# lionl1106/Searchable-Generative-Image-Compression

Measured on AMD Instinct MI355X. Metric: images/sec end-to-end compress (enc+entropy+CLIP) at 256x256, higher is better.
Workload: dtype f32; 1 GPU; configs[1]: batch=32 256x256 encoder+entropy+CLIP compress per GPU, TiTok ViT-L hybrid encoder + ViT-B/32 CLIP, synthetic weights; global_batch=32

## Files before the change

### include/sgic.h

```cpp
#ifndef SGIC_H
#define SGIC_H
#include <stddef.h>
#include <stdint.h>

#ifdef __cplusplus
extern "C" {
#endif

typedef struct ihipStream_t *sgic_stream_t;

#define SGIC_OK 0
#define SGIC_EINVAL -1
#define SGIC_EHIP -2
#define SGIC_ENOSPC -3
#define SGIC_ENODEV -4

const char *sgic_last_error(void);
int sgic_version(void);
int sgic_device_count(void);


int sgic_pmf_to_quantized_cdf(const float *pmf, int n, int precision, uint32_t *cdf_out);

typedef struct sgic_cdf_table sgic_cdf_table;
// ... 38 lines not shown
  int attn_mode;
  sgic_profiler *profiler;
  int w_packed;
  int a_packed;
} sgic_launch_opts;

int sgic_profiler_create(sgic_profiler **out);
void sgic_profiler_destroy(sgic_profiler *p);
int sgic_profiler_begin(sgic_profiler *p, int max_launches);
int sgic_profiler_end(sgic_profiler *p, float *ms_out, int cap, int *n_out);

int sgic_gemm_f32(const float *d_A, int lda, const float *d_W, int ldw, const float *d_bias, const float *d_R,
                  int ldr, float *d_C, int ldc, int M, int N, int K, int act, int a_seg, int a_seg_stride,
                  int c_seg, int c_seg_stride, const sgic_launch_opts *opts, sgic_stream_t stream);

int sgic_layernorm_f32(const float *d_x, int ldx, int xseg, int xseg_stride, const float *d_gamma,
                       const float *d_beta, float *d_y, int ldy, int yseg, int yseg_stride, int M, int C, float eps,
                       int act, sgic_stream_t stream);

int sgic_attention_f32(const float *d_q, int ldq, const float *d_k, int ldk, const float *d_v, int ldv,
                       float *d_out, int ldo, int L, int nseq, int nheads, const int32_t *d_rowmap,
                       const float *d_bias, const int32_t *d_biasvar, float scale, const sgic_launch_opts *opts,
                       sgic_stream_t stream);

int sgic_im2col_patch(const float *d_x, int B, int C, int H, int W, int P, float mul, float add, int tile16,
                      float *d_out, sgic_stream_t stream);
int sgic_assemble_tokens(const float *d_emb, const float *d_cls, const float *d_pos, const float *d_lat,
                         const float *d_latpos, int N, int P, int T, int D, float *d_out, sgic_stream_t stream);
int sgic_add_rows_bcast(const float *d_in, int ldi, int iseg, const float *d_vec, float *d_out, int ldo, int oseg,
                        int Nn, int Lr, int D, sgic_stream_t stream);
int sgic_dwconv_nhwc(const float *d_x, const float *d_w, const float *d_bias, const float *d_prescale, float *d_y,
                     int B, int H, int W, int C, int k, int tile16, sgic_stream_t stream);
int sgic_im2col_2x2(const float *d_x, int B, int H, int W, int C, int tile16, float *d_out, sgic_stream_t stream);
int sgic_gated_lrelu(const float *d_x, float *d_out, int M, int C2, sgic_stream_t stream);
int sgic_colop(const float *d_x, int ldx, const float *d_v, int ldv, int vrows, float *d_y, int ldy, int M, int C,
               int mode, sgic_stream_t stream);
int sgic_fake2d_transpose(const float *d_in, long in_seq_stride, float *d_out, int N, int T, int D,
                          sgic_stream_t stream);
int sgic_vq_argmin(const float *d_z, int ldz, const float *d_codebook, int ncodes, int dim, int M, int l2norm,
                   int32_t *d_idx, sgic_stream_t stream);
int sgic_clip_preprocess(const float *d_x, long img_stride, long ch_stride, int ldx, int B, int H, int W, int OH,
                         int OW, int S, int top, int left, const int32_t *d_bounds_h, const int32_t *d_kk_h,
                         int ksize_h, const int32_t *d_bounds_v, const int32_t *d_kk_v, int ksize_v,
                         const float *mean3, const float *std3, uint8_t *d_tmp_u8, uint8_t *d_tmp_h, float *d_out,
                         sgic_stream_t stream);
int sgic_l2norm_u8(const float *d_x, int ldx, int M, int D, float *d_unit, uint8_t *d_q, sgic_stream_t stream);

int sgic_split3_f32(const float *d_x, int ld, int rows, int cols, int seg, int seg_stride, uint16_t *d_planes,
                    sgic_stream_t stream);
int sgic_split3_pack_f32(const float *d_x, int ld, int rows, int cols, uint16_t *d_planes, sgic_stream_t stream);
int sgic_gemm_split3_f32(const float *d_A, int lda, int a_seg, int a_seg_stride, uint16_t *d_Aplanes,
                         const uint16_t *d_Wplanes, const float *d_bias, const float *d_R, int ldr, float *d_C, int ldc,
                         uint16_t *d_Cplanes, int M, int N, int K, int act, int c_seg, int c_seg_stride,
                         const sgic_launch_opts *opts, sgic_stream_t stream);
int sgic_conv3x3_split3_f32(const uint16_t *d_in_planes, const uint16_t *d_Wplanes, const float *d_bias, const float *d_R,
                            int ldr, float *d_out, int ldc, int B, int H, int W, int Cin, int Cout, int act,
                            const sgic_launch_opts *opts, sgic_stream_t stream);
int sgic_groupnorm_nhwc_split3(const float *d_x, const float *d_gamma, const float *d_beta, int B, int H, int W, int C,
                               int groups, float eps, int swish, double *d_ws, float *d_stats, uint16_t *d_halo_planes,
                               sgic_stream_t stream);
int sgic_halo_copy_split3(const float *d_in, int B, int H, int W, int C, int upsample2x, int tile16, uint16_t *d_halo_planes,
                          sgic_stream_t stream);
int sgic_attention_split3_f32(const float *d_q, int ldq, const float *d_k, int ldk, const float *d_v, int ldv,
                              uint16_t *d_out_planes, long rows, int L, int nseq, int nheads, const int32_t *d_rowmap,
                              const float *d_bias, const int32_t *d_biasvar, float scale, const sgic_launch_opts *opts,
                              sgic_stream_t stream);
int sgic_layernorm_split3_f32(const float *d_x, int ldx, int xseg, int xseg_stride, const float *d_gamma,
                              const float *d_beta, uint16_t *d_planes, int M, int C, float eps, int act,
                              sgic_stream_t stream);

int sgic_gemm_batched_f32(const float *d_A, int lda, long strideA, const float *d_W, int ldw, long strideW,
                          const float *d_bias, const float *d_R, int ldr, long strideR, float *d_C, int ldc,
                          long strideC, int M, int N, int K, int act, int batch, const sgic_launch_opts *opts,
                          sgic_stream_t stream);
int sgic_conv3x3_f32(const float *d_in_halo, const float *d_W, const float *d_bias, const float *d_R, int ldr,
                     float *d_out, int ldc, int B, int H, int W, int Cin, int Cout, int act, const sgic_launch_opts *opts,
                     sgic_stream_t stream);
int sgic_groupnorm_nhwc(const float *d_x, const float *d_gamma, const float *d_beta, int B, int H, int W, int C,
                        int groups, float eps, int swish, int halo_out, double *d_ws, float *d_stats, float *d_y,
                        sgic_stream_t stream);
int sgic_halo_copy(const float *d_in, int B, int H, int W, int C, int upsample2x, int tile16, float *d_out,
                   sgic_stream_t stream);
int sgic_softmax_rows(const float *d_x, float *d_y, long M, int L, float scale, sgic_stream_t stream);
int sgic_pixel_shuffle2_tm16(const float *d_in, int B, int H, int W, int C, float *d_out, sgic_stream_t stream);
int sgic_assemble_dec_tokens(const float *d_emb, const float *d_cls, const float *d_mask, const float *d_pos,
                             const float *d_latpos, int N, int P, int T, int D, float *d_out, sgic_stream_t stream);
int sgic_codebook_gather_norm(const int32_t *d_idx, const float *d_codebook, int M, int dim, int ld, float *d_out,
                              sgic_stream_t stream);
int sgic_nhwc3_to_nchw_clamp(const float *d_in, int ld, int B, int H, int W, float *d_out, sgic_stream_t stream);
// ... 50 lines not shown
```

### searchable-generative-image-compression_amd/clip.py

```python
import math

import numpy as np
import torch

from . import ops
from ._lib import call
from .config import ClipConfig
from .encoder import RabW, rab_forward

_PREC = 22


def _bicubic(x):
    a = -0.5
    x = abs(x)
    if x < 1.0:
        return ((a + 2.0) * x - (a + 3.0)) * x * x + 1
    if x < 2.0:
        return (((x - 5) * x + 8) * x - 4) * a
    return 0.0


def pil_coeffs(in_size, out_size):
    scale = in_size / out_size
    fscale = max(scale, 1.0)
    support = 2.0 * fscale
    ksize = int(math.ceil(support)) * 2 + 1
    bounds = np.zeros((out_size, 2), dtype=np.int32)
    kk = np.zeros((out_size, ksize), dtype=np.int32)
    ss = 1.0 / fscale
    for xx in range(out_size):
# ... 5 lines not shown
        w = [_bicubic((x + xmin - center + 0.5) * ss) for x in range(xmax)]
        ww = 0.0
        for v in w:
            ww += v
        if ww != 0.0:
            w = [v / ww for v in w]
        for x, v in enumerate(w):
            kk[xx, x] = int(-0.5 + v * (1 << _PREC)) if v < 0 else int(0.5 + v * (1 << _PREC))
        bounds[xx] = (xmin, xmax)
    return bounds, kk, ksize


def resize_geometry(H, W, S):
    if H <= W:
        OH, OW = S, int(S * W / H)
    else:
        OH, OW = int(S * H / W), S
    top = int(round((OH - S) / 2.0))
    left = int(round((OW - S) / 2.0))
    return OH, OW, top, left


class ClipHIP:
    def __init__(self, sd, cfg: ClipConfig, device, p="clip.visual"):
        self.cfg, self.device = cfg, device
        g = lambda k: sd[f"{p}.{k}"].to(device=device, dtype=torch.float32).contiguous()
        Wd = cfg.width
        self.conv_w = sd[f"{p}.conv1.weight"].reshape(Wd, -1).to(device).contiguous()
        self.cls = g("class_embedding").reshape(1, Wd).contiguous()
        self.pos = g("positional_embedding")
        self.lnpre_w, self.lnpre_b = g("ln_pre.weight"), g("ln_pre.bias")
        self.blocks = [RabW(sd, f"{p}.transformer.resblocks.{i}", device) for i in range(cfg.layers)]
        self.lnpost_w, self.lnpost_b = g("ln_post.weight"), g("ln_post.bias")
        self.projT = sd[f"{p}.proj"].t().to(device).contiguous()
        self.mean = np.asarray(cfg.mean, dtype=np.float32)
        self.std = np.asarray(cfg.std, dtype=np.float32)
        self._coef = {}

    def _coeffs(self, H, W):
        key = (H, W)
        if key not in self._coef:
            S = self.cfg.image_size
            OH, OW, top, left = resize_geometry(H, W, S)
            bh, kh, ksh = pil_coeffs(W, OW)
            bv, kv, ksv = pil_coeffs(H, OH)
            d = lambda a: torch.from_numpy(np.ascontiguousarray(a)).to(self.device)
            self._coef[key] = (OH, OW, top, left, d(bh), d(kh), ksh, d(bv), d(kv), ksv)
        return self._coef[key]
# ... 31 lines not shown
             self.mean, self.std, ops._p(work), ctypes.c_size_t(nbytes.value), ops._p(out))
        return out

    def preprocess_u8(self, canvas, hw):
        if canvas.dim() != 4 or canvas.shape[3] != 3 or canvas.dtype != torch.uint8:
            raise ValueError(f"canvas must be (B, Hc, Wc, 3) uint8, got {tuple(canvas.shape)} {canvas.dtype}")
        B, Hc, Wc, _ = canvas.shape
        hw = np.asarray(hw, dtype=np.int64).reshape(B, 2)
        if (hw <= 0).any() or (hw[:, 0] > Hc).any() or (hw[:, 1] > Wc).any():
            raise ValueError(f"extents {hw.tolist()} outside the {Hc}x{Wc} canvas")
        S = self.cfg.image_size
        geo = np.array([(h, w) + resize_geometry(h, w, S) for h, w in hw.tolist()], dtype=np.int32)
        return ops.clip_preprocess_u8canvas(canvas.contiguous(), geo, S, self.mean, self.std)

    def tower(self, pre):
        cfg = self.cfg
        B = pre.shape[0]
        g = cfg.image_size // cfg.patch
        L = g * g + 1
        A = ops.im2col_patch(pre, cfg.patch, 1.0, 0.0, tile16=False)
        emb = ops.gemm(A, self.conv_w)
        X = ops.assemble_tokens(emb, self.cls, self.pos, None, None, B, g * g, 0, cfg.width)
        ops.layernorm(X, self.lnpre_w, self.lnpre_b, out=X)
        for w in self.blocks:
            rab_forward(X, w, L, B, cfg.heads)
        pooled = ops.layernorm(X, self.lnpost_w, self.lnpost_b, M=B, x_seg=(1, L))
        z = ops.gemm(pooled, self.projT)
        return ops.l2norm_u8(z)

    def encode(self, x, H=None, W=None, hw=None):
        return self.tower(self.preprocess(x, H, W, hw))

    def encode_u8(self, canvas, hw):
        return self.tower(self.preprocess_u8(canvas, hw))


class ClipTextHIP:

    def __init__(self, sd, cfg: ClipConfig, device, p="clip"):
        self.cfg, self.device = cfg, device
        g = lambda k: sd[f"{p}.{k}"].to(device=device, dtype=torch.float32).contiguous()
        self.table, self.pos = g("token_embedding.weight"), g("positional_embedding")
        self.blocks = [RabW(sd, f"{p}.transformer.resblocks.{i}", device) for i in range(cfg.t_layers)]
        self.lnf_w, self.lnf_b = g("ln_final.weight"), g("ln_final.bias")
        self.projT = sd[f"{p}.text_projection"].t().to(device=device, dtype=torch.float32).contiguous()
        L = self.L = (cfg.ctx + 3) & ~3
        if L != cfg.ctx:
            self.pos = torch.cat([self.pos, torch.zeros(L - cfg.ctx, cfg.t_width, device=device)]).contiguous()
        self.causal = torch.full((L, L), float("-inf")).triu_(1).reshape(1, L, L).to(device).contiguous()
# ... 20 lines not shown
```

### searchable-generative-image-compression_amd/csrc/attn.hip

```cpp
#include "common.h"
#include "split3.h"

typedef float f32x16 __attribute__((ext_vector_type(16)));
typedef float f32x4 __attribute__((ext_vector_type(4)));

#define AT_KT 32
#define AT_LOG2E 1.4426950408889634f
#define AT_DEFER 6.0f
#define AT_LDK 68
#define AT_LDV 64
#define AT_TILE (AT_KT * AT_LDK + AT_KT * AT_LDV)
#define AT_K3_ROWB 144
#define AT_K3_FLOATS (3 * AT_KT * AT_K3_ROWB / 4)
#define AT_V3_ROWB 80
#define AT_V3_FLOATS (3 * 64 * AT_V3_ROWB / 4)
typedef __bf16 at_bf16x8 __attribute__((ext_vector_type(8)));
typedef unsigned at_u32x4 __attribute__((ext_vector_type(4)));
typedef unsigned at_u32x2 __attribute__((ext_vector_type(2)));
#define AT_RAG_MAXL 960
#define AT_RAG_SLICE (64 + AT_RAG_MAXL)

#ifdef AT_STAMPS
__device__ long long at_stamps[4 * (1 << 17)];
__device__ long long at_real[2 * (1 << 17)];
// ... 9 lines not shown
#define AT_STAMP(i)
#endif

struct AttnArgs {
  const float *q, *k, *v;
  float *out;
  int ldq, ldk, ldv, ldo;
  int L, nseq, nheads;
  const int *rowmap;
  const float *bias;
  const int *biasvar;
  float scale;
  int nq;
  int ipw;
  int nqp;
  int n_items;
  int n_wgs;
  int group;
  int rag;
  int n_rag_wgs;
  int stagger_cycles, first_round;
  unsigned short *out_planes;
  long plane_elems;
};

__device__ __forceinline__ long at_row(const AttnArgs &a, int seq, int tok) {
  return a.rowmap ? (long)a.rowmap[(long)seq * a.L + tok] : (long)seq * a.L + tok;
}

__device__ void attn_ragged_row(const AttnArgs &a, int unit, int tok, float *wl , int lane) {
  const int head = unit % a.nheads, seq = unit / a.nheads, hc = head * 64;
  const long q_row = at_row(a, seq, tok);
  float *ql = wl, *pl = wl + 64;
  ql[lane] = a.q[q_row * a.ldq + hc + lane] * a.scale;
  const float *bias_row = nullptr;
  if (a.bias) bias_row = a.bias + ((long)(a.biasvar ? a.biasvar[seq] : 0) * a.L + tok) * a.L;
  float mx = -INFINITY;
  for (int key = lane; key < a.L; key += 64) {
    const float *kp = a.k + at_row(a, seq, key) * a.ldk + hc;
    float sc = 0.f;
#pragma unroll
    for (int c = 0; c < 16; c += 4) {
      f32x4 k4[4];
#pragma unroll
      for (int j = 0; j < 4; j++) k4[j] = *reinterpret_cast<const f32x4 *>(kp + (c + j) * 4);
#pragma unroll
      for (int j = 0; j < 4; j++) {
        const f32x4 q4 = *reinterpret_cast<const f32x4 *>(ql + (c + j) * 4);
#pragma unroll
        for (int t = 0; t < 4; t++) sc = fmaf(k4[j][t], q4[t], sc);
      }
    }
    if (bias_row) sc += bias_row[key];
    pl[key] = sc;
    mx = fmaxf(mx, sc);
// ... 27 lines not shown
    s3_split_pair(res, 0.f, p1, p2, p3);
    const size_t dst = s3_pack_off(q_row, hc + lane, a.plane_elems / (a.nheads * 64));
    a.out_planes[dst] = (unsigned short)p1;
    a.out_planes[a.plane_elems + dst] = (unsigned short)p2;
    a.out_planes[2 * a.plane_elems + dst] = (unsigned short)p3;
  } else {
    a.out[q_row * a.ldo + hc + lane] = res;
  }
}

static_assert(4 * AT_RAG_SLICE <= AT_TILE, "ragged-row slices must fit the smallest LDS configuration");

template <int NBUF, int UP, bool S3>
__global__ __launch_bounds__(256, (NBUF * UP >= 4 || (S3 && UP > 1)) ? 2 : 3) void attn_f32_kernel(AttnArgs a) {
  constexpr int KF = S3 ? AT_K3_FLOATS : AT_KT * AT_LDK;
  constexpr int VF = S3 ? AT_V3_FLOATS : AT_KT * AT_LDV;
  constexpr int TILE = KF + VF;
  __shared__ __attribute__((aligned(16))) float smem[NBUF * UP * TILE];
  const int tid = threadIdx.x, lane = tid & 63, wave = tid >> 6;

  int p = blockIdx.x;
  if (p < a.n_rag_wgs) {
    const int it = p * 4 + wave, n_units = a.nseq * a.nheads;
    if (it < n_units * a.rag) attn_ragged_row(a, it / a.rag, a.nq * 32 + it % a.rag, smem + wave * AT_RAG_SLICE, lane);
    return;
  }
  p -= a.n_rag_wgs;
  const int wg = (((p >> 3) / a.group) * 8 + (p & 7)) * a.group + (p >> 3) % a.group;
  if (wg >= a.n_wgs) return;

  if (a.stagger_cycles > 0 && p < a.first_round) {
    const unsigned slot = __builtin_amdgcn_s_getreg((3 << 11) | 4) & 7u;
    const unsigned s0 = __builtin_amdgcn_readfirstlane(slot);
    if (s0 > 0) {
      const long long t_end = (long long)__builtin_amdgcn_s_memtime() + (long long)s0 * a.stagger_cycles;
      while ((long long)__builtin_amdgcn_s_memtime() < t_end) __builtin_amdgcn_s_sleep(32);
    }
  }

  AT_STAMP(0);
  const int item0 = wg * a.ipw;
  const int uA = item0 / a.nqp;
  const int last = min(item0 + a.ipw, a.n_items) - 1;
  const bool two = UP > 1 && (last / a.nqp) != uA;
  const int item = item0 + wave;
  const int unit_i = item / a.nqp, rb_i = item - unit_i * a.nqp;
  const bool active = wave < a.ipw && item < a.n_items && rb_i < a.nq;
  const int unit = active ? unit_i : uA;
  const int rb = active ? rb_i : 0;
  const int mine = (UP > 1 && unit != uA) ? 1 : 0;
  const int head = unit % a.nheads, seq = unit / a.nheads;

  const int lq = lane & 31, lh = lane >> 5;
  const int q_tok = rb * 32 + lq;
  const bool q_ok = active && q_tok < a.L;
  const int q_tok_c = q_tok < a.L ? q_tok : a.L - 1;
  const long q_row = at_row(a, seq, q_tok_c);
  const int hc = head * 64;

  float qf[S3 ? 1 : 32];
  at_bf16x8 q3[S3 ? 4 : 1][3];
  {
    const float *qp = a.q + q_row * a.ldq + hc;
    if constexpr (S3) {
#pragma unroll
      for (int c = 0; c < 4; c++) {
        const f32x4 v0 = *reinterpret_cast<const f32x4 *>(qp + 16 * c + 8 * lh), v1 = *reinterpret_cast<const f32x4 *>(qp + 16 * c + 8 * lh + 4);
        at_u32x4 p1, p2, p3;
        unsigned a0, b0, c0;
        const float qs = a.scale * AT_LOG2E;
        s3_split_pair(v0[0] * qs, v0[1] * qs, a0, b0, c0); p1[0] = a0, p2[0] = b0, p3[0] = c0;
        s3_split_pair(v0[2] * qs, v0[3] * qs, a0, b0, c0); p1[1] = a0, p2[1] = b0, p3[1] = c0;
        s3_split_pair(v1[0] * qs, v1[1] * qs, a0, b0, c0); p1[2] = a0, p2[2] = b0, p3[2] = c0;
        s3_split_pair(v1[2] * qs, v1[3] * qs, a0, b0, c0); p1[3] = a0, p2[3] = b0, p3[3] = c0;
        q3[c][0] = __builtin_bit_cast(at_bf16x8, p1);
        q3[c][1] = __builtin_bit_cast(at_bf16x8, p2);
        q3[c][2] = __builtin_bit_cast(at_bf16x8, p3);
      }
    } else {
#pragma unroll
// ... 334 lines not shown
#pragma unroll
      for (int t = 0; t < 4; t++) w0[t] = o0[g4 * 4 + t] * inv, w1[t] = o1[g4 * 4 + t] * inv;
      if (a.out_planes) {
        const size_t prows = a.plane_elems / (a.nheads * 64);
        const size_t dst = s3_pack_off(q_row, hc + d, prows);
        s3_store4(a.out_planes, a.plane_elems, dst, w0);
        s3_store4(a.out_planes, a.plane_elems, dst + prows * 32, w1);
      } else {
        *reinterpret_cast<f32x4 *>(op + d) = w0;
        *reinterpret_cast<f32x4 *>(op + 32 + d) = w1;
      }
    }
  }
  AT_STAMP(3);
}

template <typename K>
static inline void launch_attn(K kernel, unsigned grid, hipStream_t st, const AttnArgs &a) {
  kernel<<<grid, 256, 0, st>>>(a);
}

static int attention_any(const float *d_q, int ldq, const float *d_k, int ldk, const float *d_v, int ldv, float *d_out, int ldo,
                         uint16_t *d_planes, long plane_rows, int L, int nseq, int nheads, const int32_t *d_rowmap,
                         const float *d_bias, const int32_t *d_biasvar, float scale, const sgic_launch_opts *opts,
                         sgic_stream_t stream) {
  SGIC_REQUIRE(d_q && d_k && d_v && (d_out || d_planes) && L > 0 && nseq > 0 && nheads > 0, "args");
  SGIC_REQUIRE((ldq & 3) == 0 && (ldk & 3) == 0 && (ldv & 3) == 0 && (ldo & 3) == 0, "row strides must be multiples of 4");
  SGIC_REQUIRE(ldq >= nheads * 64 && ldk >= nheads * 64 && ldv >= nheads * 64 && (d_planes || ldo >= nheads * 64), "head_dim is 64");
  SGIC_REQUIRE((((uintptr_t)d_q | (uintptr_t)d_k | (uintptr_t)d_v | (uintptr_t)d_out) & 15) == 0 && ((uintptr_t)d_planes & 7) == 0, "16-byte alignment");
  SGIC_REQUIRE(!d_planes || plane_rows >= (long)nseq * L, "plane rows");
  SGIC_REQUIRE(!d_bias || (L & 3) == 0, "bias needs L % 4 == 0");
  const int mode_all = opts ? opts->attn_mode : 0;
  SGIC_REQUIRE(mode_all >= 0 && mode_all <= 15, "attn_mode 0..7 (+8)");
  const bool s3 = (mode_all & 8) != 0;
  const int mode = mode_all & 7;
  const long units = (long)nseq * nheads;
  const int rem = L % 32;
  const int rag = (rem >= 1 && rem <= 2 && L >= 64 && L <= AT_RAG_MAXL) ? rem : 0;
  const int nq = rag ? L / 32 : (L + 31) / 32;
  const bool three = mode == 7 && nq >= 2;
  const int ipw = three ? 3 : (nq == 1 ? 2 : 4);
  const int nqp = three ? (nq + 2) / 3 * 3 : nq;
  const long n_items = units * nqp;
  SGIC_REQUIRE(n_items < (1l << 30), "too many (sequence, head, row block) items");
  const int n_wgs = (int)((n_items + ipw - 1) / ipw);
  const int group = (4 * nqp) / ipw;
  const long groups = (n_wgs + group - 1) / group;
  const long grid_mfma = ((groups + 7) / 8) * 8 * group;
  const int n_rag_wgs = (int)((units * rag + 3) / 4);
  const bool up2 = (nqp % ipw) != 0;
  AttnArgs a{d_q, d_k, d_v, d_out, ldq, ldk, ldv, ldo, L, nseq, nheads, d_rowmap, d_bias, d_biasvar, scale,
             nq, ipw, nqp, (int)n_items, n_wgs, group, rag, n_rag_wgs, 0, 0, d_planes, plane_rows * nheads * 64};
  const unsigned grid = (unsigned)(grid_mfma + n_rag_wgs);
  hipStream_t st = to_stream(stream);
  const int eff = three ? 1 : (mode ? (mode == 7 ? 1 : mode) : (up2 ? 5 : 1));
  const bool single = (eff & 1) != 0;
  a.stagger_cycles = eff > 2 ? 4096 * ((eff - 1) / 2) : 0;
  const int per_cu = (!single && up2) ? 2 : 3;
  a.first_round = per_cu * 256;
  if (s3) {
    if (up2) {
      if (single) launch_attn(attn_f32_kernel<1, 2, true>, grid, st, a);
      else launch_attn(attn_f32_kernel<2, 2, true>, grid, st, a);
    } else {
      if (single) launch_attn(attn_f32_kernel<1, 1, true>, grid, st, a);
      else launch_attn(attn_f32_kernel<2, 1, true>, grid, st, a);
    }
  } else if (up2) {
    if (single) launch_attn(attn_f32_kernel<1, 2, false>, grid, st, a);
    else launch_attn(attn_f32_kernel<2, 2, false>, grid, st, a);
  } else {
    if (single) launch_attn(attn_f32_kernel<1, 1, false>, grid, st, a);
    else launch_attn(attn_f32_kernel<2, 1, false>, grid, st, a);
  }
  return sgic::check_launch("attn_f32_kernel");
}

extern "C" int sgic_attention_f32(const float *d_q, int ldq, const float *d_k, int ldk, const float *d_v, int ldv,
                                  float *d_out, int ldo, int L, int nseq, int nheads, const int32_t *d_rowmap,
                                  const float *d_bias, const int32_t *d_biasvar, float scale, const sgic_launch_opts *opts,
                                  sgic_stream_t stream) {
  SGIC_REQUIRE(d_out, "out");
  return attention_any(d_q, ldq, d_k, ldk, d_v, ldv, d_out, ldo, nullptr, 0, L, nseq, nheads, d_rowmap, d_bias, d_biasvar, scale,
                       opts, stream);
}

extern "C" int sgic_attention_split3_f32(const float *d_q, int ldq, const float *d_k, int ldk, const float *d_v, int ldv,
                                         uint16_t *d_out_planes, long rows, int L, int nseq, int nheads,
                                         const int32_t *d_rowmap, const float *d_bias, const int32_t *d_biasvar, float scale,
                                         const sgic_launch_opts *opts, sgic_stream_t stream) {
  SGIC_REQUIRE(d_out_planes, "planes");
  return attention_any(d_q, ldq, d_k, ldk, d_v, ldv, nullptr, 0, d_out_planes, rows, L, nseq, nheads, d_rowmap, d_bias, d_biasvar,
                       scale, opts, stream);
}
```

### searchable-generative-image-compression_amd/csrc/misc.hip

```cpp
#include "common.h"
#include <limits.h>

typedef float f32x4 __attribute__((ext_vector_type(4)));

__device__ __forceinline__ long fmap_row(int b, int y, int x, int H, int W, int tile16) {
  if (!tile16) return ((long)b * H + y) * W + x;
  const int nH = H >> 4, nW = W >> 4;
  return ((((long)b * nH + (y >> 4)) * nW + (x >> 4)) << 8) + ((y & 15) << 4) + (x & 15);
}

#define GRID_STRIDE(i, n) for (long i = (long)blockIdx.x * blockDim.x + threadIdx.x; i < (n); i += (long)gridDim.x * blockDim.x)
static inline unsigned ew_grid(long n) {
  long g = (n + 255) / 256;
  return (unsigned)(g < 1 ? 1 : (g > 8192 ? 8192 : g));
}

__global__ void im2col_patch_kernel(const float *__restrict__ x, int B, int C, int H, int W, int P, float mul, float add,
                                    int tile16, float *__restrict__ out) {
  const int gh = H / P, gw = W / P, K = C * P * P, P4 = P >> 2;
  const long total = (long)B * gh * gw * C * P * P4;
  GRID_STRIDE(i, total) {
    long t = i;
    const int kx4 = (int)(t % P4);
    t /= P4;
// ... 242 lines not shown
  SGIC_REQUIRE(d_x && d_v && d_y && M > 0 && C > 0 && (C & 3) == 0 && vrows > 0 && (mode >= 0 && mode <= 2), "args");
  SGIC_REQUIRE((ldx & 3) == 0 && (ldv & 3) == 0 && (ldy & 3) == 0, "leading dims multiple of 4");
  colop_kernel<<<ew_grid((long)M * C / 4), 256, 0, to_stream(stream)>>>(d_x, ldx, d_v, ldv, vrows, d_y, ldy, M, C, mode);
  return sgic::check_launch("colop_kernel");
}

__global__ void fake2d_transpose_kernel(const float *__restrict__ in, long in_seq_stride, float *__restrict__ out, int N,
                                        int T, int D) {
  const long total = (long)N * T * D;
  GRID_STRIDE(i, total) {
    const int c = (int)(i % D);
    const long r = i / D;
    const int t = (int)(r % T);
    const int n = (int)(r / T);
    out[i] = in[(long)n * in_seq_stride + (long)c * T + t];
  }
}

extern "C" int sgic_fake2d_transpose(const float *d_in, long in_seq_stride, float *d_out, int N, int T, int D,
                                     sgic_stream_t stream) {
  SGIC_REQUIRE(d_in && d_out && N > 0 && T > 0 && D > 0, "args");
  fake2d_transpose_kernel<<<ew_grid((long)N * T * D), 256, 0, to_stream(stream)>>>(d_in, in_seq_stride, d_out, N, T, D);
  return sgic::check_launch("fake2d_transpose_kernel");
}

#define VQ_TPW 4
__global__ __launch_bounds__(256) void vq_argmin_kernel(const float *__restrict__ z, int ldz, const float *__restrict__ cb,
                                                        int ncodes, int dim, int M, int l2norm, int *__restrict__ idx) {
  __shared__ float s_z[VQ_TPW][17];
  __shared__ float s_best[4][VQ_TPW];
  __shared__ int s_besti[4][VQ_TPW];
  const int tid = threadIdx.x, lane = tid & 63, wave = tid >> 6;
  const int m0 = blockIdx.x * VQ_TPW;
  if (tid < VQ_TPW) {
    const int m = min(m0 + tid, M - 1);
    float zv[16];
    float zn = 0.f;
#pragma unroll
    for (int d = 0; d < 16; d++) {
      zv[d] = d < dim ? z[(long)m * ldz + d] : 0.f;
      if (d < dim) zn += zv[d] * zv[d];
    }
    if (l2norm) {
      const float inv = 1.0f / fmaxf(sqrtf(zn), 1e-12f);
      zn = 0.f;
#pragma unroll
// ... 699 lines not shown
```

### searchable-generative-image-compression_amd/encoder.py

```python
import numpy as np
import torch

from . import ops
from .config import CodecConfig


def _dev(t, device):
    return t.to(device=device, dtype=torch.float32).contiguous()


class RabW:

    def __init__(self, sd, p, device):
        g = lambda k: _dev(sd[f"{p}.{k}"], device)
        self.ln1w, self.ln1b = g("ln_1.weight"), g("ln_1.bias")
        self.inw, self.inb = g("attn.in_proj_weight"), g("attn.in_proj_bias")
        self.ow, self.ob = g("attn.out_proj.weight"), g("attn.out_proj.bias")
        self.ln2w, self.ln2b = g("ln_2.weight"), g("ln_2.bias")
        self.fcw, self.fcb = g("mlp.c_fc.weight"), g("mlp.c_fc.bias")
        self.pjw, self.pjb = g("mlp.c_proj.weight"), g("mlp.c_proj.bias")


def rab_forward(X, w: RabW, L, nseq, heads, bias=None):
    D = X.shape[1]
    h = ops.layernorm(X, w.ln1w, w.ln1b, to_gemm=True)
    qkv = ops.gemm(h, w.inw, w.inb)
    att = ops.attention(qkv[:, 0:D], qkv[:, D:2 * D], qkv[:, 2 * D:3 * D], h, L, nseq, heads, bias=bias, to_gemm=True)
    ops.gemm(att, w.ow, w.ob, residual=X, out=X)
    h = ops.layernorm(X, w.ln2w, w.ln2b, out=h, to_gemm=True)
    f = ops.gemm(h, w.fcw, w.fcb, act=ops.ACT_GELU, to_gemm=True)
    ops.gemm(f, w.pjw, w.pjb, residual=X, out=X)
    return X


def rel_indices(win):
    idx = torch.tensor([[x, y] for x in range(win) for y in range(win)])
    return idx[None, :, :] - idx[:, None, :] + win - 1


class SwinW:

    def __init__(self, sd, p, shifted, rel, win, device):
        g = lambda k: _dev(sd[f"{p}.{k}"], device)
        self.shifted = shifted
        self.n1w, self.n1b = g("norm_attn.weight"), g("norm_attn.bias")
        self.qkvw = g("attention_block.to_qkv.weight")
        self.ow, self.ob = g("attention_block.to_out.weight"), g("attention_block.to_out.bias")
        self.n2w, self.n2b = g("norm_mlp.weight"), g("norm_mlp.bias")
        self.w0, self.b0 = g("mlp_block.net.0.weight"), g("mlp_block.net.0.bias")
        self.w2, self.b2 = g("mlp_block.net.2.weight"), g("mlp_block.net.2.bias")
        pos = sd[f"{p}.attention_block.pos_embedding"].float()
        if rel:
            ri = rel_indices(win)
            pos = pos[ri[:, :, 0], ri[:, :, 1]]
        if shifted:
# ... 79 lines not shown
        self.fw, self.fb = g("feat_add.1.weight"), g("feat_add.1.bias")
        self.zw, self.zb = g("zero_add.weight"), g("zero_add.bias")


def cross_forward(Fm, X, w: CrossW, N, Lt, P2):
    Fd = Fm.shape[1]
    LJ = Lt + P2
    J = torch.empty(N * LJ, Fd, device=X.device, dtype=torch.float32)
    tmp = torch.empty_like(X)
    ops.add_rows_bcast(X, Lt, w.tpos, tmp, Lt, N, Lt)
    ops.gemm(tmp, w.cw, w.cb, out=J, M=N * Lt, c_seg=(Lt, LJ))
    ops.add_rows_bcast(Fm, P2, w.fpos, J[Lt:], LJ, N, P2)
    for rw in w.attn:
        rab_forward(J, rw, LJ, N, Fd // 64)
    t = ops.layernorm(J[Lt:], w.fnw, w.fnb, M=N * P2, x_seg=(P2, LJ), to_gemm=True)
    ops.gemm(t, w.fw, w.fb, residual=Fm, out=Fm)
    t = ops.gemm(J, w.dw, w.db, M=N * Lt, a_seg=(Lt, LJ))
    t = ops.layernorm(t, w.dnw, w.dnb, out=t, act=ops.ACT_SILU, to_gemm=True)
    ops.gemm(t, w.zw, w.zb, residual=X, out=X)
    return Fm, X


class HybridEncoderHIP:
    def __init__(self, sd, cfg: CodecConfig, device, p="hybrid_codec.encoder"):
        self.cfg, self.device = cfg, device
        g = lambda k: _dev(sd[f"{p}.{k}"], device)
        Wd, Fd = cfg.width, cfg.feat_dim
        self.pe_w = _dev(sd[f"{p}.patch_embed.weight"].reshape(Wd, -1), device)
        self.pe_b = g("patch_embed.bias")
        self.cls, self.pos, self.latpos = g("class_embedding"), g("positional_embedding"), g("latent_token_positional_embedding")
        self.lat = _dev(sd["hybrid_codec.latent_tokens"], device)
        self.lnpre_w, self.lnpre_b = g("ln_pre.weight"), g("ln_pre.bias")
        self.layers = [RabW(sd, f"{p}.transformer.{i}", device) for i in range(cfg.layers)]
        self.lnpost_w, self.lnpost_b = g("ln_post.weight"), g("ln_post.bias")
        self.co_w = _dev(sd[f"{p}.conv_out.weight"].reshape(cfg.token_size, Wd), device)
        self.co_b = g("conv_out.bias")
        self.pix_w = _dev(sd[f"{p}.pix_emb_proj.weight"].reshape(Fd, Wd), device)
        self.pix_b = g("pix_emb_proj.bias")
        self.cross, self.fblocks = {}, {}
        for i in cfg.in_pos_enc:
            self.cross[i] = CrossW(sd, f"{p}.inter_blocks.{i}", cfg.n_attn, device)
            self.fblocks[i] = (swin_stack_weights(sd, f"{p}.feat_blocks.{i}.0", 2, cfg.window, device),
                               ConvNextW(sd, f"{p}.feat_blocks.{i}.1", device), ConvNextW(sd, f"{p}.feat_blocks.{i}.2", device))
        self.feat_in = swin_stack_weights(sd, f"{p}.feat_in", 4, cfg.window, device)
        self.feat_out_swin = swin_stack_weights(sd, f"{p}.feat_out.0", 2, cfg.window, device)
        self.fo_cw = _dev(sd[f"{p}.feat_out.1.weight"].permute(0, 2, 3, 1).reshape(Fd, 4 * Fd), device)
        self.fo_cb = g("feat_out.1.bias")
        self.fo_nw, self.fo_nb = g("feat_out.3.weight"), g("feat_out.3.bias")
        self.fo_lw, self.fo_lb = g("feat_out.4.weight"), g("feat_out.4.bias")

    def forward(self, x, taps=None):
        cfg = self.cfg
        B, _, H, W = x.shape
        P, g, T, Wd = cfg.patch_size, cfg.grid, cfg.num_latent_tokens, cfg.width
        Hf, Wf = H // P, W // P
        nH, nW = Hf // g, Wf // g
        N, P2 = B * nH * nW, g * g
        L = 1 + P2 + T
        A = ops.im2col_patch(x, P, 0.5, 0.5, tile16=True)
        emb = ops.gemm(A, self.pe_w, self.pe_b)
        Fm = ops.gemm(emb, self.pix_w, self.pix_b)
        X = ops.assemble_tokens(emb, self.cls, self.pos, self.lat, self.latpos, N, P2, T, Wd)
        for w in self.feat_in:
            swin_forward(Fm, w, B, Hf, Wf, cfg.window)
        ops.layernorm(X, self.lnpre_w, self.lnpre_b, out=X)
        if taps is not None:
            taps["feat_in"] = Fm.clone()
            taps["x_ln_pre"] = X.clone()
        for i in range(cfg.layers):
            rab_forward(X, self.layers[i], L, N, cfg.heads)
            if i in self.cross:
                cross_forward(Fm, X, self.cross[i], N, 1 + P2 + T, P2)
                sw, c1, c2 = self.fblocks[i]
                for w in sw:
                    swin_forward(Fm, w, B, Hf, Wf, cfg.window)
                convnext_forward(Fm, c1, B, Hf, Wf)
                convnext_forward(Fm, c2, B, Hf, Wf)
            if taps is not None and i == 0:
                taps["x_layer0"] = X.clone()
        lat = ops.layernorm(X[1 + P2:], self.lnpost_w, self.lnpost_b, M=N * T, x_seg=(T, L))
        latT = ops.fake2d_transpose(lat, T * Wd, N, T, Wd)
        z = ops.gemm(latT, self.co_w, self.co_b)
        for w in self.feat_out_swin:
            swin_forward(Fm, w, B, Hf, Wf, cfg.window)
        A2 = ops.im2col_2x2(Fm, B, Hf, Wf, tile16=True)
        h = ops.gemm(A2, self.fo_cw, self.fo_cb)
        ops.layernorm(h, self.fo_nw, self.fo_nb, out=h)
        h = ops.gemm(h, self.fo_lw, self.fo_lb)
        return z, h, (nH, nW)
```

### searchable-generative-image-compression_amd/ops.py

```python
import ctypes
import json
import os

import numpy as np
import torch

from ._lib import call, check, launch_opts, lib, require_gpu

ACT_NONE, ACT_GELU, ACT_SILU, ACT_TANH, ACT_LRELU = 0, 1, 2, 3, 4

PROFILE = None
_PROFILER = None


def _profiler():
    global _PROFILER
    if _PROFILER is None:
        h = ctypes.c_void_p(0)
        check(lib.sgic_profiler_create(ctypes.byref(h)), "sgic_profiler_create")
        _PROFILER = h
    return _PROFILER


def profile_begin(max_launches=8192):
# ... 440 lines not shown


def layernorm(x, gamma, beta, out=None, eps=1e-5, act=ACT_NONE, M=None, x_seg=(0, 0), y_seg=(0, 0), to_gemm=False):
    x, ldx = _rows(x)
    C = x.shape[1]
    if M is None:
        M = x.shape[0]
    assert gamma.shape == (C,) and beta.shape == (C,)
    if to_gemm and planes_ok(C) and C % 256 == 0 and C <= 2048 and y_seg[0] == 0:
        pl = out if isinstance(out, Planes) and out.shape == (M, C) else Planes(M, C, x.device, buf=out.t if isinstance(out, Planes) else None)
        call("sgic_layernorm_split3_f32", _p(x), ldx, x_seg[0], x_seg[1], _p(gamma), _p(beta), _p(pl.t), M, C, float(eps), act)
        return pl
    if isinstance(out, Planes):
        out = None
    if out is None:
        assert y_seg[0] == 0
        out = torch.empty(M, C, device=x.device, dtype=torch.float32)
    out, ldy = _rows(out)
    call("sgic_layernorm_f32", _p(x), ldx, x_seg[0], x_seg[1], _p(gamma), _p(beta), _p(out), ldy, y_seg[0], y_seg[1],
         M, C, float(eps), act)
    return out


def attention(q, k, v, out, L, nseq, nheads, rowmap=None, bias=None, biasvar=None, scale=0.125, mode=None, to_gemm=False, precision=None):
    q, ldq = _rows(q)
    k, ldk = _rows(k)
    v, ldv = _rows(v)
    D = nheads * 64
    pl = None
    if to_gemm and planes_ok(D):
        rows = q.shape[0]
        pl = out if isinstance(out, Planes) and out.shape == (rows, D) else Planes(rows, D, q.device, buf=out.t if isinstance(out, Planes) else None)
    else:
        if out is None or isinstance(out, Planes):
            out = torch.empty(q.shape[0], D, device=q.device, dtype=torch.float32)
        out, ldo = _rows(out)
    if rowmap is not None:
        assert rowmap.dtype == torch.int32 and rowmap.numel() == nseq * L and rowmap.is_contiguous()
    if bias is not None:
        assert bias.dim() == 3 and bias.shape[1] == L and bias.shape[2] == L and bias.is_contiguous()
    if biasvar is not None:
        assert biasvar.dtype == torch.int32 and biasvar.numel() == nseq

    s3 = 8 if (precision or PRECISION) == "split3" else 0

    def launch(m):
        if pl is not None:
            call("sgic_attention_split3_f32", _p(q), ldq, _p(k), ldk, _p(v), ldv, _p(pl.t), ctypes.c_long(pl.rows), L, nseq, nheads,
                 _p(rowmap), _p(bias), _p(biasvar), float(scale), launch_opts(0, m | s3, None))
        else:
            call("sgic_attention_f32", _p(q), ldq, _p(k), ldk, _p(v), ldv, _p(out), ldo, L, nseq, nheads, _p(rowmap), _p(bias),
                 _p(biasvar), float(scale), launch_opts(0, m | s3, None))

    if mode is None:
        mode = 0
        if nseq * nheads * L >= 4096:
            key = ("attn3" if s3 else "attn", nseq, L, nheads, int(bias is not None))
            mode = _lookup(key)
            if mode is None:
                mode = 0
                if AUTOTUNE and PROFILE is None:
                    best_t = None
                    for cand in ATTN_MODES:
                        launch(cand)
                        e0, e1 = torch.cuda.Event(enable_timing=True), torch.cuda.Event(enable_timing=True)
                        e0.record()
                        for _ in range(3):
                            launch(cand)
                        e1.record()
                        e1.synchronize()
                        t = e0.elapsed_time(e1)
                        if best_t is None or t < best_t:
                            mode, best_t = cand, t
                    _remember(key, mode)
    launch(mode)
    return pl if pl is not None else out


def im2col_patch(x, P, mul=1.0, add=0.0, tile16=False, out=None):
    assert x.dim() == 4 and x.is_contiguous() and x.dtype == torch.float32
    B, C, H, W = x.shape
    if out is None:
        out = torch.empty(B * (H // P) * (W // P), C * P * P, device=x.device, dtype=torch.float32)
    call("sgic_im2col_patch", _p(x), B, C, H, W, P, float(mul), float(add), int(tile16), _p(out))
    return out


def assemble_tokens(emb, cls, pos, lat, latpos, N, P, T, D, out=None):
    if out is None:
        out = torch.empty(N * (1 + P + T), D, device=emb.device, dtype=torch.float32)
    call("sgic_assemble_tokens", _p(emb), _p(cls), _p(pos), _p(lat), _p(latpos), N, P, T, D, _p(out))
    return out


def add_rows_bcast(inp, iseg, vec, out, oseg, Nn, Lr):
    inp, ldi = _rows(inp)
    out, ldo = _rows(out)
    D = inp.shape[1]
    assert out.shape[1] == D
    if vec is not None:
        assert vec.is_contiguous() and vec.numel() == Lr * D
# ... 426 lines not shown
```

Before: 511.6 images/s.

## Prune last transformer block to only the rows consumed downstream

In the last transformer block of both the TiTok encoder and the CLIP visual tower, only the query rows that are actually read afterwards are computed: latent tokens plus one for the encoder, and the first 32 rows, keeping only CLS, for CLIP. K/V are still computed over the full sequence. Queries, attention, output projection and MLP run on the reduced row set. This uses a new windowed attention entry point and a strided block-copy helper. The aim is to drop wasted compute on patch-token rows in the final layer, at the cost of extra kernels and a separate layernorm over the query rows.

```diff
diff --git a/include/sgic.h b/include/sgic.h
--- a/include/sgic.h
+++ b/include/sgic.h
@@ -84,6 +84,12 @@
                        float *d_out, int ldo, int L, int nseq, int nheads, const int32_t *d_rowmap,
                        const float *d_bias, const int32_t *d_biasvar, float scale, const sgic_launch_opts *opts,
                        sgic_stream_t stream);
+int sgic_attention_window_f32(const float *d_q, int ldq, const float *d_k, int ldk, const float *d_v, int ldv,
+                              float *d_out, int ldo, int L, int nseq, int nheads, const int32_t *d_rowmap,
+                              const float *d_bias, const int32_t *d_biasvar, float scale, int q_tok0, int Lq,
+                              const sgic_launch_opts *opts, sgic_stream_t stream);
+int sgic_copy_blocks_f32(const float *d_src, long src_stride, float *d_dst, long dst_stride, long block_elems, int nblocks,
+                         sgic_stream_t stream);
 
 int sgic_im2col_patch(const float *d_x, int B, int C, int H, int W, int P, float mul, float add, int tile16,
                       float *d_out, sgic_stream_t stream);
@@ -127,6 +133,10 @@
                               uint16_t *d_out_planes, long rows, int L, int nseq, int nheads, const int32_t *d_rowmap,
                               const float *d_bias, const int32_t *d_biasvar, float scale, const sgic_launch_opts *opts,
                               sgic_stream_t stream);
+int sgic_attention_window_split3_f32(const float *d_q, int ldq, const float *d_k, int ldk, const float *d_v, int ldv,
+                                     uint16_t *d_out_planes, long rows, int L, int nseq, int nheads, const int32_t *d_rowmap,
+                                     const float *d_bias, const int32_t *d_biasvar, float scale, int q_tok0, int Lq,
+                                     const sgic_launch_opts *opts, sgic_stream_t stream);
 int sgic_layernorm_split3_f32(const float *d_x, int ldx, int xseg, int xseg_stride, const float *d_gamma,
                               const float *d_beta, uint16_t *d_planes, int M, int C, float eps, int act,
                               sgic_stream_t stream);
diff --git a/searchable-generative-image-compression_amd/clip.py b/searchable-generative-image-compression_amd/clip.py
--- a/searchable-generative-image-compression_amd/clip.py
+++ b/searchable-generative-image-compression_amd/clip.py
@@ -6,7 +6,7 @@
 from . import ops
 from ._lib import call
 from .config import ClipConfig
-from .encoder import RabW, rab_forward
+from .encoder import RabW, rab_forward, rab_forward_last
 
 _PREC = 22
 
@@ -58,8 +58,9 @@
 
 
 class ClipHIP:
-    def __init__(self, sd, cfg: ClipConfig, device, p="clip.visual"):
+    def __init__(self, sd, cfg: ClipConfig, device, p="clip.visual", prune_last=True):
         self.cfg, self.device = cfg, device
+        self.prune_last = prune_last
         g = lambda k: sd[f"{p}.{k}"].to(device=device, dtype=torch.float32).contiguous()
         Wd = cfg.width
         self.conv_w = sd[f"{p}.conv1.weight"].reshape(Wd, -1).to(device).contiguous()
@@ -137,9 +138,15 @@
         emb = ops.gemm(A, self.conv_w)
         X = ops.assemble_tokens(emb, self.cls, self.pos, None, None, B, g * g, 0, cfg.width)
         ops.layernorm(X, self.lnpre_w, self.lnpre_b, out=X)
-        for w in self.blocks:
-            rab_forward(X, w, L, B, cfg.heads)
-        pooled = ops.layernorm(X, self.lnpost_w, self.lnpost_b, M=B, x_seg=(1, L))
+        if self.prune_last and L > 32:
+            for w in self.blocks[:-1]:
+                rab_forward(X, w, L, B, cfg.heads)
+            pooled = rab_forward_last(X, self.blocks[-1], L, B, cfg.heads, 0, 32, keep=1)
+            ops.layernorm(pooled, self.lnpost_w, self.lnpost_b, out=pooled)
+        else:
+            for w in self.blocks:
+                rab_forward(X, w, L, B, cfg.heads)
+            pooled = ops.layernorm(X, self.lnpost_w, self.lnpost_b, M=B, x_seg=(1, L))
         z = ops.gemm(pooled, self.projT)
         return ops.l2norm_u8(z)
 
diff --git a/searchable-generative-image-compression_amd/csrc/attn.hip b/searchable-generative-image-compression_amd/csrc/attn.hip
--- a/searchable-generative-image-compression_amd/csrc/attn.hip
+++ b/searchable-generative-image-compression_amd/csrc/attn.hip
@@ -55,15 +55,19 @@
   int stagger_cycles, first_round;
   unsigned short *out_planes;
   long plane_elems;
+  int q_tok0, Lq, rb0, rag_tok0;
 };
 
 __device__ __forceinline__ long at_row(const AttnArgs &a, int seq, int tok) {
   return a.rowmap ? (long)a.rowmap[(long)seq * a.L + tok] : (long)seq * a.L + tok;
 }
+__device__ __forceinline__ long at_qrow(const AttnArgs &a, int seq, int tok) {
+  return a.Lq ? (long)seq * a.Lq + (tok - a.q_tok0) : at_row(a, seq, tok);
+}
 
 __device__ void attn_ragged_row(const AttnArgs &a, int unit, int tok, float *wl , int lane) {
   const int head = unit % a.nheads, seq = unit / a.nheads, hc = head * 64;
-  const long q_row = at_row(a, seq, tok);
+  const long q_row = at_qrow(a, seq, tok);
   float *ql = wl, *pl = wl + 64;
   ql[lane] = a.q[q_row * a.ldq + hc + lane] * a.scale;
   const float *bias_row = nullptr;
@@ -137,7 +141,7 @@
   int p = blockIdx.x;
   if (p < a.n_rag_wgs) {
     const int it = p * 4 + wave, n_units = a.nseq * a.nheads;
-    if (it < n_units * a.rag) attn_ragged_row(a, it / a.rag, a.nq * 32 + it % a.rag, smem + wave * AT_RAG_SLICE, lane);
+    if (it < n_units * a.rag) attn_ragged_row(a, it / a.rag, a.rag_tok0 + it % a.rag, smem + wave * AT_RAG_SLICE, lane);
     return;
   }
   p -= a.n_rag_wgs;
@@ -162,7 +166,7 @@
   const int unit_i = item / a.nqp, rb_i = item - unit_i * a.nqp;
   const bool active = wave < a.ipw && item < a.n_items && rb_i < a.nq;
   const int unit = active ? unit_i : uA;
-  const int rb = active ? rb_i : 0;
+  const int rb = a.rb0 + (active ? rb_i : 0);
   const int mine = (UP > 1 && unit != uA) ? 1 : 0;
   const int head = unit % a.nheads, seq = unit / a.nheads;
 
@@ -170,7 +174,7 @@
   const int q_tok = rb * 32 + lq;
   const bool q_ok = active && q_tok < a.L;
   const int q_tok_c = q_tok < a.L ? q_tok : a.L - 1;
-  const long q_row = at_row(a, seq, q_tok_c);
+  const long q_row = at_qrow(a, seq, q_tok_c);
   const int hc = head * 64;
 
   float qf[S3 ? 1 : 32];
@@ -551,13 +555,13 @@
 
 static int attention_any(const float *d_q, int ldq, const float *d_k, int ldk, const float *d_v, int ldv, float *d_out, int ldo,
                          uint16_t *d_planes, long plane_rows, int L, int nseq, int nheads, const int32_t *d_rowmap,
-                         const float *d_bias, const int32_t *d_biasvar, float scale, const sgic_launch_opts *opts,
-                         sgic_stream_t stream) {
+                         const float *d_bias, const int32_t *d_biasvar, float scale, int q_tok0, int Lq,
+                         const sgic_launch_opts *opts, sgic_stream_t stream) {
   SGIC_REQUIRE(d_q && d_k && d_v && (d_out || d_planes) && L > 0 && nseq > 0 && nheads > 0, "args");
   SGIC_REQUIRE((ldq & 3) == 0 && (ldk & 3) == 0 && (ldv & 3) == 0 && (ldo & 3) == 0, "row strides must be multiples of 4");
   SGIC_REQUIRE(ldq >= nheads * 64 && ldk >= nheads * 64 && ldv >= nheads * 64 && (d_planes || ldo >= nheads * 64), "head_dim is 64");
   SGIC_REQUIRE((((uintptr_t)d_q | (uintptr_t)d_k | (uintptr_t)d_v | (uintptr_t)d_out) & 15) == 0 && ((uintptr_t)d_planes & 7) == 0, "16-byte alignment");
-  SGIC_REQUIRE(!d_planes || plane_rows >= (long)nseq * L, "plane rows");
+  SGIC_REQUIRE(!d_planes || plane_rows >= (long)nseq * (Lq ? Lq : L), "plane rows");
   SGIC_REQUIRE(!d_bias || (L & 3) == 0, "bias needs L % 4 == 0");
   const int mode_all = opts ? opts->attn_mode : 0;
   SGIC_REQUIRE(mode_all >= 0 && mode_all <= 15, "attn_mode 0..7 (+8)");
@@ -565,8 +569,18 @@
   const int mode = mode_all & 7;
   const long units = (long)nseq * nheads;
   const int rem = L % 32;
-  const int rag = (rem >= 1 && rem <= 2 && L >= 64 && L <= AT_RAG_MAXL) ? rem : 0;
-  const int nq = rag ? L / 32 : (L + 31) / 32;
+  int rag = (rem >= 1 && rem <= 2 && L >= 64 && L <= AT_RAG_MAXL) ? rem : 0;
+  int nq = rag ? L / 32 : (L + 31) / 32;
+  int rb0 = 0, rag_tok0 = nq * 32;
+  if (Lq) {
+    const int q_end = q_tok0 + Lq;
+    SGIC_REQUIRE(!d_rowmap, "a query window takes no row map");
+    SGIC_REQUIRE(q_tok0 >= 0 && (q_tok0 & 31) == 0 && Lq > 0 && q_tok0 < nq * 32, "window start: a row block of the sequence");
+    SGIC_REQUIRE(q_end >= L || (q_end & 31) == 0, "window end: a row-block boundary, or the end of the sequence");
+    rb0 = q_tok0 / 32;
+    rag = max(0, min(rag, q_end - rag_tok0));
+    nq = min(nq, (q_end + 31) / 32) - rb0;
+  }
   const bool three = mode == 7 && nq >= 2;
   const int ipw = three ? 3 : (nq == 1 ? 2 : 4);
   const int nqp = three ? (nq + 2) / 3 * 3 : nq;
@@ -579,7 +593,8 @@
   const int n_rag_wgs = (int)((units * rag + 3) / 4);
   const bool up2 = (nqp % ipw) != 0;
   AttnArgs a{d_q, d_k, d_v, d_out, ldq, ldk, ldv, ldo, L, nseq, nheads, d_rowmap, d_bias, d_biasvar, scale,
-             nq, ipw, nqp, (int)n_items, n_wgs, group, rag, n_rag_wgs, 0, 0, d_planes, plane_rows * nheads * 64};
+             nq, ipw, nqp, (int)n_items, n_wgs, group, rag, n_rag_wgs, 0, 0, d_planes, plane_rows * nheads * 64,
+             q_tok0, Lq, rb0, rag_tok0};
   const unsigned grid = (unsigned)(grid_mfma + n_rag_wgs);
   hipStream_t st = to_stream(stream);
   const int eff = three ? 1 : (mode ? (mode == 7 ? 1 : mode) : (up2 ? 5 : 1));
@@ -611,7 +626,16 @@
                                   sgic_stream_t stream) {
   SGIC_REQUIRE(d_out, "out");
   return attention_any(d_q, ldq, d_k, ldk, d_v, ldv, d_out, ldo, nullptr, 0, L, nseq, nheads, d_rowmap, d_bias, d_biasvar, scale,
-                       opts, stream);
+                       0, 0, opts, stream);
+}
+
+extern "C" int sgic_attention_window_f32(const float *d_q, int ldq, const float *d_k, int ldk, const float *d_v, int ldv,
+                                         float *d_out, int ldo, int L, int nseq, int nheads, const int32_t *d_rowmap,
+                                         const float *d_bias, const int32_t *d_biasvar, float scale, int q_tok0, int Lq,
+                                         const sgic_launch_opts *opts, sgic_stream_t stream) {
+  SGIC_REQUIRE(d_out && Lq > 0, "out / window");
+  return attention_any(d_q, ldq, d_k, ldk, d_v, ldv, d_out, ldo, nullptr, 0, L, nseq, nheads, d_rowmap, d_bias, d_biasvar, scale,
+                       q_tok0, Lq, opts, stream);
 }
 
 extern "C" int sgic_attention_split3_f32(const float *d_q, int ldq, const float *d_k, int ldk, const float *d_v, int ldv,
@@ -620,5 +644,14 @@
                                          const sgic_launch_opts *opts, sgic_stream_t stream) {
   SGIC_REQUIRE(d_out_planes, "planes");
   return attention_any(d_q, ldq, d_k, ldk, d_v, ldv, nullptr, 0, d_out_planes, rows, L, nseq, nheads, d_rowmap, d_bias, d_biasvar,
-                       scale, opts, stream);
-}
+                       scale, 0, 0, opts, stream);
+}
+
+extern "C" int sgic_attention_window_split3_f32(const float *d_q, int ldq, const float *d_k, int ldk, const float *d_v, int ldv,
+                                                uint16_t *d_out_planes, long rows, int L, int nseq, int nheads,
+                                                const int32_t *d_rowmap, const float *d_bias, const int32_t *d_biasvar, float scale,
+                                                int q_tok0, int Lq, const sgic_launch_opts *opts, sgic_stream_t stream) {
+  SGIC_REQUIRE(d_out_planes && Lq > 0, "planes / window");
+  return attention_any(d_q, ldq, d_k, ldk, d_v, ldv, nullptr, 0, d_out_planes, rows, L, nseq, nheads, d_rowmap, d_bias, d_biasvar,
+                       scale, q_tok0, Lq, opts, stream);
+}
diff --git a/searchable-generative-image-compression_amd/csrc/misc.hip b/searchable-generative-image-compression_amd/csrc/misc.hip
--- a/searchable-generative-image-compression_amd/csrc/misc.hip
+++ b/searchable-generative-image-compression_amd/csrc/misc.hip
@@ -288,6 +288,15 @@
   SGIC_REQUIRE(d_in && d_out && N > 0 && T > 0 && D > 0, "args");
   fake2d_transpose_kernel<<<ew_grid((long)N * T * D), 256, 0, to_stream(stream)>>>(d_in, in_seq_stride, d_out, N, T, D);
   return sgic::check_launch("fake2d_transpose_kernel");
+}
+
+extern "C" int sgic_copy_blocks_f32(const float *d_src, long src_stride, float *d_dst, long dst_stride, long block_elems,
+                                    int nblocks, sgic_stream_t stream) {
+  SGIC_REQUIRE(d_src && d_dst && block_elems > 0 && nblocks > 0, "args");
+  SGIC_REQUIRE(src_stride >= block_elems && dst_stride >= block_elems, "strides");
+  SGIC_HIP(hipMemcpy2DAsync(d_dst, (size_t)dst_stride * 4, d_src, (size_t)src_stride * 4, (size_t)block_elems * 4, (size_t)nblocks,
+                            hipMemcpyDeviceToDevice, to_stream(stream)));
+  return SGIC_OK;
 }
 
 #define VQ_TPW 4
diff --git a/searchable-generative-image-compression_amd/encoder.py b/searchable-generative-image-compression_amd/encoder.py
--- a/searchable-generative-image-compression_amd/encoder.py
+++ b/searchable-generative-image-compression_amd/encoder.py
@@ -31,6 +31,27 @@
     f = ops.gemm(h, w.fcw, w.fcb, act=ops.ACT_GELU, to_gemm=True)
     ops.gemm(f, w.pjw, w.pjb, residual=X, out=X)
     return X
+
+
+def rab_forward_last(X, w: RabW, L, nseq, heads, tok0, Lq, keep=None, bias=None):
+    D = X.shape[1]
+    keep = Lq if keep is None else keep
+    assert 0 < keep <= Lq and tok0 + Lq <= L
+    h = ops.layernorm(X, w.ln1w, w.ln1b, to_gemm=True)
+    kv = ops.gemm(h, w.inw[D:], w.inb[D:])
+    hq = ops.layernorm(X[tok0:], w.ln1w, w.ln1b, M=nseq * Lq, x_seg=(Lq, L), to_gemm=True)
+    q = ops.gemm(hq, w.inw[:D], w.inb[:D])
+    Xq = ops.copy_row_blocks(X[tok0:], keep, L, nseq)
+    if keep == Lq:
+        att = ops.attention(q, kv[:, 0:D], kv[:, D:2 * D], hq, L, nseq, heads, bias=bias, to_gemm=True, window=(tok0, Lq))
+        ops.gemm(att, w.ow, w.ob, residual=Xq, out=Xq)
+    else:
+        att = ops.attention(q, kv[:, 0:D], kv[:, D:2 * D], None, L, nseq, heads, bias=bias, window=(tok0, Lq))
+        ops.gemm(att, w.ow, w.ob, residual=Xq, out=Xq, M=nseq * keep, a_seg=(keep, Lq))
+    h = ops.layernorm(Xq, w.ln2w, w.ln2b, to_gemm=True)
+    f = ops.gemm(h, w.fcw, w.fcb, act=ops.ACT_GELU, to_gemm=True)
+    ops.gemm(f, w.pjw, w.pjb, residual=Xq, out=Xq)
+    return Xq
 
 
 def rel_indices(win):
@@ -156,8 +177,9 @@
 
 
 class HybridEncoderHIP:
-    def __init__(self, sd, cfg: CodecConfig, device, p="hybrid_codec.encoder"):
+    def __init__(self, sd, cfg: CodecConfig, device, p="hybrid_codec.encoder", prune_last=True):
         self.cfg, self.device = cfg, device
+        self.prune_last = prune_last
         g = lambda k: _dev(sd[f"{p}.{k}"], device)
         Wd, Fd = cfg.width, cfg.feat_dim
         self.pe_w = _dev(sd[f"{p}.patch_embed.weight"].reshape(Wd, -1), device)
@@ -201,7 +223,9 @@
         if taps is not None:
             taps["feat_in"] = Fm.clone()
             taps["x_ln_pre"] = X.clone()
-        for i in range(cfg.layers):
+        last = cfg.layers - 1
+        prune = self.prune_last and taps is None and last not in self.cross and P2 % 32 == 0
+        for i in range(cfg.layers - 1 if prune else cfg.layers):
             rab_forward(X, self.layers[i], L, N, cfg.heads)
             if i in self.cross:
                 cross_forward(Fm, X, self.cross[i], N, 1 + P2 + T, P2)
@@ -212,7 +236,11 @@
                 convnext_forward(Fm, c2, B, Hf, Wf)
             if taps is not None and i == 0:
                 taps["x_layer0"] = X.clone()
-        lat = ops.layernorm(X[1 + P2:], self.lnpost_w, self.lnpost_b, M=N * T, x_seg=(T, L))
+        if prune:
+            Xq = rab_forward_last(X, self.layers[last], L, N, cfg.heads, P2, T + 1)
+            lat = ops.layernorm(Xq[1:], self.lnpost_w, self.lnpost_b, M=N * T, x_seg=(T, T + 1))
+        else:
+            lat = ops.layernorm(X[1 + P2:], self.lnpost_w, self.lnpost_b, M=N * T, x_seg=(T, L))
         latT = ops.fake2d_transpose(lat, T * Wd, N, T, Wd)
         z = ops.gemm(latT, self.co_w, self.co_b)
         for w in self.feat_out_swin:
diff --git a/searchable-generative-image-compression_amd/ops.py b/searchable-generative-image-compression_amd/ops.py
--- a/searchable-generative-image-compression_amd/ops.py
+++ b/searchable-generative-image-compression_amd/ops.py
@@ -486,7 +486,8 @@
     return out
 
 
-def attention(q, k, v, out, L, nseq, nheads, rowmap=None, bias=None, biasvar=None, scale=0.125, mode=None, to_gemm=False, precision=None):
+def attention(q, k, v, out, L, nseq, nheads, rowmap=None, bias=None, biasvar=None, scale=0.125, mode=None, to_gemm=False, precision=None,
+              window=None):
     q, ldq = _rows(q)
     k, ldk = _rows(k)
     v, ldv = _rows(v)
@@ -501,6 +502,11 @@
         out, ldo = _rows(out)
     if rowmap is not None:
         assert rowmap.dtype == torch.int32 and rowmap.numel() == nseq * L and rowmap.is_contiguous()
+    q_tok0, Lq = window if window is not None else (0, 0)
+    if window is not None:
+        assert Lq > 0 and q.shape[0] >= nseq * Lq and (pl is not None or out.shape[0] >= nseq * Lq), (window, q.shape)
+    win = "_window" if window is not None else ""
+    wargs = (int(q_tok0), int(Lq)) if window is not None else ()
     if bias is not None:
         assert bias.dim() == 3 and bias.shape[1] == L and bias.shape[2] == L and bias.is_contiguous()
     if biasvar is not None:
@@ -510,16 +516,16 @@
 
     def launch(m):
         if pl is not None:
-            call("sgic_attention_split3_f32", _p(q), ldq, _p(k), ldk, _p(v), ldv, _p(pl.t), ctypes.c_long(pl.rows), L, nseq, nheads,
-                 _p(rowmap), _p(bias), _p(biasvar), float(scale), launch_opts(0, m | s3, None))
+            call(f"sgic_attention{win}_split3_f32", _p(q), ldq, _p(k), ldk, _p(v), ldv, _p(pl.t), ctypes.c_long(pl.rows), L, nseq, nheads,
+                 _p(rowmap), _p(bias), _p(biasvar), float(scale), *wargs, launch_opts(0, m | s3, None))
         else:
-            call("sgic_attention_f32", _p(q), ldq, _p(k), ldk, _p(v), ldv, _p(out), ldo, L, nseq, nheads, _p(rowmap), _p(bias),
-                 _p(biasvar), float(scale), launch_opts(0, m | s3, None))
+            call(f"sgic_attention{win}_f32", _p(q), ldq, _p(k), ldk, _p(v), ldv, _p(out), ldo, L, nseq, nheads, _p(rowmap), _p(bias),
+                 _p(biasvar), float(scale), *wargs, launch_opts(0, m | s3, None))
 
     if mode is None:
         mode = 0
         if nseq * nheads * L >= 4096:
-            key = ("attn3" if s3 else "attn", nseq, L, nheads, int(bias is not None))
+            key = ("attn3" if s3 else "attn", nseq, L, nheads, int(bias is not None)) + wargs
             mode = _lookup(key)
             if mode is None:
                 mode = 0
@@ -541,6 +547,17 @@
     return pl if pl is not None else out
 
 
+def copy_row_blocks(x, rows, stride_rows, nblocks, out=None):
+    x, ldx = _rows(x)
+    C = x.shape[1]
+    assert ldx == C and stride_rows >= rows and x.shape[0] >= (nblocks - 1) * stride_rows + rows, (x.shape, rows, stride_rows, nblocks)
+    if out is None:
+        out = torch.empty(nblocks * rows, C, device=x.device, dtype=torch.float32)
+    assert out.is_contiguous() and out.shape == (nblocks * rows, C)
+    call("sgic_copy_blocks_f32", _p(x), _cl(stride_rows * C), _p(out), _cl(rows * C), _cl(rows * C), nblocks)
+    return out
+
+
 def im2col_patch(x, P, mul=1.0, add=0.0, tile16=False, out=None):
     assert x.dim() == 4 and x.is_contiguous() and x.dtype == torch.float32
     B, C, H, W = x.shape
```

Measured after the change: 517.2 images/s, median of 6. +1.1%, better.
